# taylor-santos/RelativityPathTracer

Measured on AMD Instinct MI355X. Metric: Mrays/s (primary rays) on Scenes/bunny.txt at 3840x2160, higher is better.
Workload: dtype f32

## Files before the change

include/rpt.h:

```cpp
#ifndef RPT_H
#define RPT_H

#include "rpt_layout.h"

#ifdef __cplusplus
extern "C" {
#endif

typedef struct rpt_ctx rpt_ctx;

enum rpt_status {
    RPT_OK = 0,
    RPT_ERR_ARG = 1,
    RPT_ERR_STATE = 2,
    RPT_ERR_SCENE = 3,
    RPT_ERR_DEVICE = 4,
    RPT_ERR_NOMEM = 5
};

#define RPT_TILE_ROWS 8
#define RPT_LATENCY_KERNEL_MAX_PIXELS 3000000

const char *rpt_version(void);

// ... 39 lines not shown
int rpt_raymap_fill(int kind, const float *params, int width, int height, float *dirs3_out);

int rpt_set_environment(rpt_ctx *ctx, const unsigned char *rgb8, int width, int height);
int rpt_set_environment_frame(rpt_ctx *ctx, const float lorentz[16]);

int rpt_set_orientation(rpt_ctx *ctx, const float ypr[3]);
int rpt_set_field_of_view(rpt_ctx *ctx, float v_fov);
int rpt_orient_objects(const void *objects_in, int count, const float ypr[3], void *objects_out);
int rpt_orient_matrix(const float lorentz_in[16], const float ypr[3], float lorentz_out[16]);

int rpt_set_variant(rpt_ctx *ctx, int variant);
int rpt_set_msaa(rpt_ctx *ctx, int samples_per_axis);
int rpt_last_variant(const rpt_ctx *ctx);
int rpt_last_exact_rcp(const rpt_ctx *ctx);
int rpt_last_sky_split(const rpt_ctx *ctx, int rect[4]);
int rpt_scene_exact_rcp(const rpt_scene_desc *s);

int rpt_verify_frame(rpt_ctx *ctx, unsigned long long *differing_pixels);

int rpt_object_screen_rect(const void *object, int interval, const float *root_bounds_or_null, float rect_out[4]);
int rpt_object_screen_bounds(const void *object, int interval, const float *root_bounds_or_null, float bounds_out[8]);
int rpt_mesh_segment_cull_record(rpt_ctx *ctx, int object_index, float out[10]);
int rpt_object_screen_bounds_proposed(const void *object, int interval, const float *root_bounds_or_null, float bounds_out[8]);
int rpt_certify_screen_bounds(const void *object, int interval, const float *root_bounds_or_null, const float bounds[8], int stats_out[4]);
int rpt_tile_bitmap_host(const rpt_scene_desc *scene, int object_index, int interval, int width, int height, float lens_scale, int max_boxes,
                         const float *boxes_or_null, int n_boxes, uint32_t *bits_out, size_t words, int stats_out[5]);
int rpt_tile_bitmap_stage_host(const rpt_scene_desc *scene, int object_index, int interval, int width, int height, float lens_scale, int stage,
                               int max_triangles, uint32_t *bits_out, size_t words, int stats_out[4]);
int rpt_tile_rasterise_host(int width, int height, float lens_scale, int diagonals, const float bounds[8], uint32_t *bits_out, size_t words);
int rpt_tile_bitmap_state(rpt_ctx *ctx, unsigned long long out[4], int object_index, uint32_t *bits_or_null, size_t words);
// ... 152 lines not shown
```

relativitypathtracer_amd/_ffi.py:

```python
from __future__ import annotations

import ctypes as C
import os

_HERE = os.path.dirname(os.path.abspath(__file__))


class Float2(C.Structure):
    _fields_ = [("x", C.c_float), ("y", C.c_float)]


class Float4(C.Structure):
    _fields_ = [("x", C.c_float), ("y", C.c_float), ("z", C.c_float), ("w", C.c_float)]


class Object(C.Structure):
    _fields_ = [
        ("M", Float4 * 4), ("InvM", Float4 * 4), ("Lorentz", Float4 * 4), ("InvLorentz", Float4 * 4),
        ("stationaryCam", Float4), ("color", Float4),
        ("type", C.c_int32), ("meshIndex", C.c_int32), ("textureIndex", C.c_int32),
        ("textureWidth", C.c_int32), ("textureHeight", C.c_int32),
        ("light", C.c_uint8), ("_pad", C.c_uint8 * 3),
        ("flashPeriod", C.c_float), ("flashDuration", C.c_float),
    ]
# ... 133 lines not shown
    "rpt_object_screen_bounds_proposed": (C.c_int, [C.c_void_p, C.c_int, C.POINTER(C.c_float), C.POINTER(C.c_float)]),
    "rpt_certify_screen_bounds": (C.c_int, [C.c_void_p, C.c_int, C.POINTER(C.c_float), C.POINTER(C.c_float), C.POINTER(C.c_int)]),
    "rpt_tile_bitmap_host": (C.c_int, [C.c_void_p, C.c_int, C.c_int, C.c_int, C.c_int, C.c_float, C.c_int, C.c_void_p, C.c_int, C.c_void_p, C.c_size_t,
                                       C.POINTER(C.c_int)]),
    "rpt_tile_bitmap_stage_host": (C.c_int, [C.c_void_p, C.c_int, C.c_int, C.c_int, C.c_int, C.c_float, C.c_int, C.c_int, C.c_void_p, C.c_size_t,
                                             C.POINTER(C.c_int)]),
    "rpt_tile_rasterise_host": (C.c_int, [C.c_int, C.c_int, C.c_float, C.c_int, C.POINTER(C.c_float), C.c_void_p, C.c_size_t]),
    "rpt_tile_bitmap_shared_state": (C.c_int, [C.c_void_p, C.POINTER(C.c_uint64)]),
    "rpt_tile_bitmap_state": (C.c_int, [C.c_void_p, C.POINTER(C.c_uint64), C.c_int, C.c_void_p, C.c_size_t]),
    "rpt_derived_layout_host": (C.c_int, [C.c_void_p, C.c_int, C.c_void_p, C.c_size_t, C.POINTER(C.c_size_t)]),
    "rpt_probe_tile_masks": (C.c_int, [C.c_void_p, C.c_void_p, C.c_size_t]),
    "rpt_verify_frame": (C.c_int, [C.c_void_p, C.POINTER(C.c_uint64)]),
    "rpt_last_variant": (C.c_int, [C.c_void_p]),
    "rpt_last_exact_rcp": (C.c_int, [C.c_void_p]),
    "rpt_last_sky_split": (C.c_int, [C.c_void_p, C.POINTER(C.c_int)]),
    "rpt_scene_exact_rcp": (C.c_int, [C.c_void_p]),
    "rpt_probe_reciprocal": (C.c_int, [C.c_void_p, C.c_float, C.c_float, C.POINTER(C.c_uint64), C.c_void_p, C.c_int]),
    "rpt_set_msaa": (C.c_int, [C.c_void_p, C.c_int]),
    "rpt_probe_walk": (C.c_int, [C.c_void_p, C.c_int, C.c_void_p, C.c_void_p, C.c_int]),
    "rpt_timing_end_spans": (C.c_int, [C.c_void_p, C.c_void_p, C.POINTER(C.c_float), C.POINTER(C.c_float), C.c_int, C.POINTER(C.c_int)]),
    "rpt_probe_object": (C.c_int, [C.c_void_p, C.c_int, C.c_int, C.c_void_p, C.c_void_p, C.c_int]),
    "rpt_render": (C.c_int, [C.c_void_p]),
    "rpt_render_async": (C.c_int, [C.c_void_p]),
    "rpt_sync": (C.c_int, [C.c_void_p]),
    "rpt_output_ptr": (C.c_void_p, [C.c_void_p]),
    "rpt_output_bytes": (C.c_size_t, [C.c_void_p]),
    "rpt_read_framebuffer": (C.c_int, [C.c_void_p, C.c_void_p, C.c_size_t]),
    "rpt_read_debug_rgb": (C.c_int, [C.c_void_p, C.c_void_p, C.c_size_t]),
    "rpt_last_frame_ms": (C.c_int, [C.c_void_p, C.POINTER(C.c_float)]),
    "rpt_timed_frames": (C.c_int, [C.c_void_p, C.c_int, C.POINTER(C.c_float)]),
# ... 145 lines not shown
```

relativitypathtracer_amd/csrc/rpt_api.hip:

```cpp
#include <hip/hip_runtime.h>

#include <cmath>
#include <cstdio>
#include <chrono>
#include <cstdlib>
#include <cstring>
#include <algorithm>
#include <atomic>
#include <functional>
#include <map>
#include <memory>
#include <mutex>
#include <string>
#include <utility>
#include <vector>

#include "../../include/rpt.h"
#include "rpt_kernels.hip.h"
#include "rpt_octree_build.hip.h"
#include "rpt_screen_bounds.hpp"
#include "rpt_bounds_certify.hpp"
#include "rpt_tile_bitmap.hpp"
#include "rpt_sky_split.hpp"
#include "rpt_workers.hpp"
// ... 131 lines not shown
    DeviceBuffer tile_masks;
    DeviceBuffer verify_planes;
    DeviceBuffer claim_counters;
    int cu_count = 0;
    unsigned int claim_epoch = 0;
    std::vector<uint8_t> host_objects;
    DeviceBuffer dobjs;
    std::vector<rptb::Rect> rects;
    int rect_interval = 0x7fffffff;
    unsigned long long rect_geo_generation = ~0ull;
    DeviceBuffer owned_out, owned_plane, owned_rgb;
    void *pinned_objects = nullptr;
    size_t pinned_capacity = 0;
    hipEvent_t staging_done[4] = {nullptr, nullptr, nullptr, nullptr};
    unsigned int staging_used = 0, staging_next = 0;
    int object_count = 0;
    bool scene_uploaded = false;

    float white_point[3] = {1, 1, 1};
    float ambient = 1.0f;
    int width = 0, height = 0, interval = -1;
    bool params_set = false;

    void *external_out = nullptr;
    void *external_plane = nullptr;
    void *external_rgb = nullptr;
    std::vector<hipEvent_t> timing_events;
    int timing_frames = -1;
    bool want_owned_rgb = false;
    int first_tile = 0, tile_step = 1, run_log2 = 0;
// ... 756 lines not shown
    const long long want = (band + sky + 3) / 4;
    static const int wgs_per_cu = std::getenv("RPT_WGS_PER_CU") ? std::atoi(std::getenv("RPT_WGS_PER_CU")) : 5;
    const unsigned int wgs = (unsigned int)std::max(1ll, std::min((long long)ctx->cu_count * wgs_per_cu, want));
    switch (v) {
    case 60: hipLaunchKernelGGL(rptd::rpt_render_kernel_persistent_w5, dim3(wgs), dim3(256), 0, ctx->stream, a, a.out16, a.plane, a.debug_rgb, claims); break;
    case 62: hipLaunchKernelGGL(rptd::rpt_render_kernel_persistent_direct_w5, dim3(wgs), dim3(256), 0, ctx->stream, a, a.out16, a.plane, a.debug_rgb, claims); break;
    case 63: hipLaunchKernelGGL(rptd::rpt_render_kernel_persistent_classic_w5, dim3(wgs), dim3(256), 0, ctx->stream, a, a.out16, a.plane, a.debug_rgb, claims); break;
    default: return fail(ctx, RPT_ERR_ARG, "unknown persistent kernel variant");
    }
    return RPT_OK;
}
#endif

#ifdef RPT_DIAGNOSTICS
#define RPT_LAUNCH_X(N) case N: hipLaunchKernelGGL(rptd::rpt_render_kernel_x##N, grid, dim3(256), 0, ctx->stream, a); break;
void launch_sky_fill(rpt_ctx *ctx, const rptd::KernelArgs &a, int tiles, const int box[4]);
int launch_diagnostic(rpt_ctx *ctx, rptd::KernelArgs &a, dim3 grid, int tiles, int v) {
    if (v == 143 || v == 2573 || (v >= 256 && v < 1000 && (v & 8))) set_band_first(ctx, a, tiles);
    switch (v) {
    case 26: {
        const int tiles_x = ((ctx->width + 31) / 32) * 4;
        const int n_tiles = tiles_x * tiles;
        if (int rc = reserve(ctx, ctx->tile_masks, (size_t)n_tiles * 8)) return rc;
        a.mask_tiles_x = tiles_x;
        a.n_tiles = n_tiles;
        a.tile_masks = (unsigned long long *)ctx->tile_masks.ptr;
        hipLaunchKernelGGL(rptd::rpt_tile_bin_kernel, dim3((n_tiles + 255) / 256), dim3(256), 0, ctx->stream, a);
        hipLaunchKernelGGL(rptd::rpt_render_kernel_v1_masked_w5, grid, dim3(256), 0, ctx->stream, a);
        break;
    }
    case 40: hipLaunchKernelGGL(rptd::rpt_render_kernel_ballot_w4, dim3(grid.x * 4, grid.y), dim3(64), 0, ctx->stream, a); break;
// ... 13 lines not shown
    case 2257: hipLaunchKernelGGL(rptd::rpt_render_kernel_x257_w4, grid, dim3(256), 0, ctx->stream, a); break;
    case 2259: hipLaunchKernelGGL(rptd::rpt_render_kernel_x259_w4, grid, dim3(256), 0, ctx->stream, a); break;
    case 2263: hipLaunchKernelGGL(rptd::rpt_render_kernel_x263_w4, grid, dim3(256), 0, ctx->stream, a); break;
    RPT_LAUNCH_X(689) RPT_LAUNCH_X(701)
    case 2573: hipLaunchKernelGGL(rptd::rpt_render_kernel_x573_w4, grid, dim3(256), 0, ctx->stream, a); break;
    case 7:
        if (int rc = reserve(ctx, ctx->counters, 16 * sizeof(unsigned long long))) return rc;
        RPT_HIP(ctx, hipMemsetAsync(ctx->counters.ptr, 0, 16 * sizeof(unsigned long long), ctx->stream));
        a.counters = (unsigned long long *)ctx->counters.ptr;
        hipLaunchKernelGGL(rptd::rpt_render_kernel_v1_diag, grid, dim3(256), 0, ctx->stream, a);
        break;
    case 8: hipLaunchKernelGGL(rptd::rpt_render_kernel_primary_only, grid, dim3(256), 0, ctx->stream, a); break;
    case 786: {
        if (!a.out16) return fail(ctx, RPT_ERR_ARG, "variant 786 writes the 16-byte framebuffer only");
        const int no_box[4] = {0, 0, 0, 0};
        launch_sky_fill(ctx, a, tiles, no_box);
        break;
    }
    case 11:
        if (int rc = reserve(ctx, ctx->wave_times, (size_t)grid.x * grid.y * 4 * 10 * sizeof(unsigned long long))) return rc;
        RPT_HIP(ctx, hipMemsetAsync(ctx->wave_times.ptr, 0, ctx->wave_times.bytes, ctx->stream));
        a.wave_times = (unsigned long long *)ctx->wave_times.ptr;
        hipLaunchKernelGGL(rptd::rpt_render_kernel_v1_timeline, grid, dim3(256), 0, ctx->stream, a);
        break;
    default: return fail(ctx, RPT_ERR_ARG, "unknown kernel variant");
    }
    return RPT_OK;
}
#endif

bool projection_params(const float *params, float out[3]) {
// ... 491 lines not shown
    if (int rc = staged_host(ctx, ctx->tile_bits, bytes, &host)) return rc;
    bool any = false;
    for (int i = 0; i < slots; i++) {
        if (!(todo >> i & 1ull)) continue;
        const auto t0 = std::chrono::steady_clock::now();
        if (!shared_tile_bitmap(ctx, objs[i], (uint32_t *)host + (size_t)i * words)) continue;
        ctx->bits_last_build_us = std::chrono::duration<double, std::micro>(std::chrono::steady_clock::now() - t0).count();
        ctx->bits_has |= 1ull << i;
        ctx->bits_builds++;
        any = true;
    }
    if (any) return staged_copy(ctx, ctx->tile_bits);
    return RPT_OK;
}

void fill_frame_args(const rpt_ctx *ctx, rptd::LensArgs &a) {
    std::memset((void *)&a, 0, sizeof a);
    a.dnodes = (const rptd::DNode *)ctx->geo->dnodes.ptr;
    a.dtris = (const rptd::DTri *)ctx->geo->dtris.ptr;
    a.links = (const int *)ctx->geo->dlinks.ptr;
    a.first_tris = (const rptd::DTri *)ctx->geo->dfirst.ptr;
    a.exits = (const rptd::DExit *)ctx->geo->dexits.ptr;
    a.hits = (const rptd::DHit *)ctx->geo->dhits.ptr;
    a.top_count = ctx->geo->top_count;
    a.dobjs = (const rptd::DObj *)((const char *)ctx->objects.ptr + (size_t)ctx->object_count * sizeof(rpt_object));
    a.objects = (const rpt_object *)ctx->objects.ptr;
    a.rects = (const float4 *)((const char *)ctx->objects.ptr + (size_t)ctx->object_count * (sizeof(rpt_object) + sizeof(rptd::DObj)));
    a.vertices = (const rpt_float3 *)ctx->geo->vertices.ptr;
    a.normals = (const rpt_float3 *)ctx->geo->normals.ptr;
    a.uvs = (const rpt_float2 *)ctx->geo->uvs.ptr;
// ... 58 lines not shown
              !rptd::tile_origin_policy<rptd::DopplerTwin<rptd::BallotExact>> && !rptd::tile_origin_policy<rptd::Lens<rptd::BallotExact>>,
              "the forms sky_split_box lets through (walk, analytic, ieee) are the kernels that add tile_x0");
bool sky_split_box(const rpt_ctx *ctx, const Choice &c, Call call, const rptd::KernelArgs &a, int tiles, int box[4]) {
    const KernelRow *row = c.colour;
    if (!row || !row->kernel || c.windowed || c.refine || row->camera != Camera::pinhole || row->colour != Colour::plain) return false;
    if (!(row->form == Form::walk || row->form == Form::analytic || row->form == Form::ieee)) return false;
    if (call.kind != CallKind::in_flight || (long long)ctx->width * ctx->height <= ctx->sky_split_min_pixels) return false;
    if (!a.out16 || a.plane || a.debug_rgb || ctx->colour_plane || ctx->first_tile != 0 || ctx->tile_step != 1 || ctx->run_log2 != 0) return false;
    if (ctx->msaa > 1 || ctx->doppler || ctx->env_on || ctx->v_fov != 0.0f || ctx->projection != RPT_PROJECTION_PINHOLE) return false;
    if (ctx->object_count < 1 || ctx->object_count > 64 || ctx->rects.size() != (size_t)ctx->object_count) return false;
    if (!rpts::object_box(ctx->rects.data(), ctx->object_count, ctx->width, ctx->height, box)) return false;
    const long long tiles_x = (ctx->width + 7) / 8, covered = (long long)(box[2] - box[0]) * (box[3] - box[1]);
    return covered * 100 <= tiles_x * tiles * ctx->sky_split_share;
}

void launch_sky_fill(rpt_ctx *ctx, const rptd::KernelArgs &a, int tiles, const int box[4]) {
    rptd::SkyFillArgs s;
    s.out16 = a.out16;
    s.width = ctx->width;
    s.height = ctx->height;
    s.bg_packed = a.bg_packed;
    s.tx0 = box[0]; s.ty0 = box[1]; s.tx1 = box[2]; s.ty1 = box[3];
    const int tiles_x = (ctx->width + 7) / 8;
    hipLaunchKernelGGL(rptd::rpt_sky_fill_kernel, dim3((tiles_x + RPT_SKY_FILL_TILES - 1) / RPT_SKY_FILL_TILES, tiles), dim3(64), 0, ctx->stream, s);
}

int launch(rpt_ctx *ctx, Call call) {
    const Choice c = choose_kernels(ctx, call);
    if (call.colour_frame && ctx->scene_uploaded && ctx->params_set) ctx->last_aa_variant = 0;
    if (c.code != RPT_OK) return fail(ctx, c.code, c.text);
    ctx->last_sky_split = false;
    if (int rc = ensure_outputs(ctx)) return rc;
    const int tiles = local_tile_count(ctx);
    if (call.colour_frame && ctx->aa_n > 1) {
        if (int rc = reserve(ctx, ctx->aa_plane, (size_t)tiles * RPT_TILE_ROWS * ctx->width * 4)) return rc;
        if (int rc = tally_ready(ctx, ctx->tally[TALLY_AA], 1)) return rc;
    }
    if (c.nothing) return RPT_OK;
    const bool panorama = ctx->projection == RPT_PROJECTION_EQUIRECT;
// ... 13 lines not shown
    a.msaa = ctx->msaa;
    a.doppler = ctx->doppler;
    a.debug_doppler = doppler_recording(ctx) ? (float *)(ctx->external_doppler ? ctx->external_doppler : ctx->owned_doppler.ptr) : nullptr;
    ctx->doppler_recorded = a.debug_doppler != nullptr;
    a.env_texels = ctx->env_on ? (const uint32_t *)ctx->env.device.ptr : nullptr;
    a.env_width = ctx->env_width;
    a.env_height = ctx->env_height;
    std::memcpy(a.env_frame, ctx->env_frame, sizeof a.env_frame);
    if (ctx->oriented) {
        rpt_float4 e[4];
        std::memcpy(e, ctx->env_frame, sizeof e);
        rebase_columns(e, ctx->R, a.env_frame);
    }

    const dim3 grid1(((ctx->width + 31) / 32) * 4, tiles);
    if (!c.colour) {
#ifdef RPT_DIAGNOSTICS
        const dim3 grid((ctx->width + 31) / 32, tiles);
        if (int rc = launch_diagnostic(ctx, a, grid, tiles, c.variant)) return rc;
#endif
    } else if (!c.colour->kernel) {
        if (rpt_launch_relaxed_kernel(relaxed_waves(c.colour->form), &a, sizeof(rptd::KernelArgs), grid1.x, grid1.y, (void *)ctx->stream)) return fail(ctx, RPT_ERR_DEVICE, "relaxed-arithmetic kernel launch failed");
    } else {
        dim3 grid = grid1;
        int box[4];
        if (sky_split_box(ctx, c, call, a, tiles, box)) {
            launch_sky_fill(ctx, a, tiles, box);
            a.tile_x0 = box[0];
            a.first_tile = box[1];
            grid = dim3(box[2] - box[0], box[3] - box[1]);
            ctx->last_sky_split = true;
            std::memcpy(ctx->last_sky_box, box, sizeof box);
        }
        void *args[] = {(void *)&a};
        (void)hipLaunchKernel(c.kernel(c.launched()), grid, dim3(64), args, 0, ctx->stream);
    }
    RPT_HIP(ctx, hipGetLastError());
    ctx->last_variant = c.variant;
    ctx->last_exact_rcp = c.ran_exact(c.launched());
    Tally &refined = ctx->tally[TALLY_AA];
    if (c.refine) {
        rptd::RefineArgs ra;
// ... 16 lines not shown
        tally_off(refined);
    }
    return RPT_OK;
}

int launch_events(rpt_ctx *ctx) {
    const Choice c = choose_kernels(ctx, Call{CallKind::events, false});
    if (c.code != RPT_OK) return fail(ctx, c.code, c.text);
    const size_t px = (size_t)ctx->width * ctx->height;
    if (!ctx->external_events && (px * sizeof(rpt_event) > ctx->owned_events.capacity || ctx->owned_events.bytes != px * sizeof(rpt_event))) {
        if (int rc = reserve(ctx, ctx->owned_events, px * sizeof(rpt_event))) return rc;
        RPT_HIP(ctx, hipMemsetAsync(ctx->owned_events.ptr, 0, px * sizeof(rpt_event), ctx->stream));
    }
    if (ctx->projection == RPT_PROJECTION_EQUIRECT)
        if (int rc = ensure_projection_tables(ctx, ctx->pano, 1)) return rc;
    rptd::RaymapEventArgs ea;
    std::memset((void *)&ea, 0, sizeof ea);
    fill_frame_args(ctx, ea);
    ea.raymap = c.colour->camera == Camera::raymap ? (const float4 *)ctx->raymap.device.ptr : nullptr;
    ea.raymap_pitch = ctx->raymap_pitch;
    ea.out16 = nullptr;
    ea.plane = nullptr;
    ea.debug_rgb = nullptr;
    ea.events = (rpt_event *)(ctx->external_events ? ctx->external_events : ctx->owned_events.ptr);
    ctx->event_frame.buffer = ea.events;
    ctx->event_frame.width = ctx->width;
    ctx->event_frame.height = ctx->height;
    ctx->events_first_tile = ctx->first_tile;
    ctx->events_tile_step = ctx->tile_step;
    ctx->events_run_log2 = ctx->run_log2;
// ... 31 lines not shown
    *out16_out = out16;
    *events_out = events;
    return RPT_OK;
}

using PassEnqueue = int (*)(rpt_ctx *ctx, Tally &tally, rpt_pixel *out16, const rpt_event *events);
int frame_pass(rpt_ctx *ctx, const char *call, bool on, int which, PassEnqueue enqueue) {
    Tally &tally = ctx->tally[which];
    if (!on) {
        tally_off(tally);
        return RPT_OK;
    }
    rpt_pixel *out16 = nullptr;
    const rpt_event *events = nullptr;
    if (int rc = frames_of_this_view(ctx, call, &out16, &events)) return rc;
    if (int rc = enqueue(ctx, tally, out16, events)) return rc;
    if (int rc = tally_home(ctx, tally)) return rc;
    ctx->last_event = tally.copied;
    return RPT_OK;
}

int enqueue_overlay(rpt_ctx *ctx, Tally &tally, rpt_pixel *out16, const rpt_event *events) {
    const rpt_overlay_desc &d = ctx->overlay;
    if (int rc = tally_ready(ctx, tally, 1, 8)) return rc;

    rptd::OverlayArgs a;
    std::memset(&a, 0, sizeof a);
    a.events = events;
    a.out16 = out16;
    a.changed = (unsigned long long *)tally.device.ptr;
// ... 405 lines not shown
const char *rpt_version(void) { return "rpt-hip 0.2 (gfx950)"; }
#endif

int rpt_create(rpt_ctx **out, int device_ordinal) {
    if (!out) return RPT_ERR_ARG;
    *out = nullptr;
    int n = 0;
    if (hipGetDeviceCount(&n) != hipSuccess || n <= 0) return RPT_ERR_DEVICE;
    if (device_ordinal < 0 || device_ordinal >= n) return RPT_ERR_ARG;
    rpt_ctx *ctx = new (std::nothrow) rpt_ctx();
    if (!ctx) return RPT_ERR_NOMEM;
    ctx->device = device_ordinal;
    ctx->tile_triangles = tile_triangles_wanted();
    ctx->sky_split_share = sky_split_share_wanted();
    ctx->sky_split_min_pixels = sky_split_min_pixels_wanted();
    (void)rpth::Workers::instance();
    {
        static std::atomic<int> created{0};
        ctx->serial = created.fetch_add(1);
    }
    ctx->geo = std::make_shared<Geometry>();
    ctx->geo->device = device_ordinal;
    if (hipSetDevice(device_ordinal) != hipSuccess || hipStreamCreateWithFlags(&ctx->own_stream, hipStreamNonBlocking) != hipSuccess ||

        hipEventCreate(&ctx->ev_begin) != hipSuccess || hipEventCreate(&ctx->ev_end) != hipSuccess) {
        rpt_destroy(ctx);
        return RPT_ERR_DEVICE;
    }
    ctx->stream = ctx->own_stream;
    if (hipDeviceGetAttribute(&ctx->cu_count, hipDeviceAttributeMultiprocessorCount, device_ordinal) != hipSuccess || ctx->cu_count <= 0) ctx->cu_count = 256;
// ... 114 lines not shown
    std::vector<uint8_t> &given = ctx->given_scratch, &turned = ctx->turned_scratch;
    given.assign((const uint8_t *)objects, (const uint8_t *)objects + bytes);
    turned.resize(bytes);
    orient_objects((const rpt_object *)given.data(), count, ctx->R, (rpt_object *)turned.data());
    const int rc = set_objects_as_given(ctx, turned.data(), count);
    if (rc == RPT_OK) ctx->caller_objects.swap(given);
    return rc;
}

static int set_objects_as_given(rpt_ctx *ctx, const void *objects, int count) {
    if (!ctx->scene_uploaded) return fail(ctx, RPT_ERR_STATE, "rpt_set_objects before rpt_upload_scene");
    RPT_HIP(ctx, hipSetDevice(ctx->device));
    if (int rc = validate_objects(ctx, (const rpt_object *)objects, count)) return rc;
    const size_t bytes = (size_t)count * sizeof(rpt_object);
    const size_t dbytes = (size_t)count * (sizeof(rptd::DObj) + sizeof(rptb::Rect));
    const size_t slot_bytes = ((bytes + dbytes + 255) / 256) * 256;
    if (slot_bytes * RPT_STAGING_SLOTS > ctx->pinned_capacity) {
        RPT_HIP(ctx, hipStreamSynchronize(ctx->stream));
        if (ctx->pinned_objects) RPT_HIP(ctx, hipHostFree(ctx->pinned_objects));
        ctx->pinned_objects = nullptr;
        ctx->pinned_capacity = 0;
        const size_t cap = (slot_bytes < 4096 ? 4096 : slot_bytes * 2) * RPT_STAGING_SLOTS;
        RPT_HIP(ctx, hipHostMalloc(&ctx->pinned_objects, cap, hipHostMallocDefault));
        ctx->pinned_capacity = cap;
        for (int k = 0; k < RPT_STAGING_SLOTS; k++)
            if (!ctx->staging_done[k]) RPT_HIP(ctx, hipEventCreateWithFlags(&ctx->staging_done[k], hipEventDisableTiming));
        ctx->staging_used = 0;
    }
    if (bytes + dbytes > ctx->objects.capacity) RPT_HIP(ctx, hipStreamSynchronize(ctx->stream));
    if (int rc = reserve(ctx, ctx->objects, bytes + dbytes)) return rc;
    if (bytes) {
        const int k = (int)(ctx->staging_next % RPT_STAGING_SLOTS);
        RPT_HOST_MARK(0);
        if (ctx->staging_used & (1u << k)) RPT_HIP(ctx, hipEventSynchronize(ctx->staging_done[k]));
        RPT_HOST_MARK(1);
        char *slot = (char *)ctx->pinned_objects + (ctx->pinned_capacity / RPT_STAGING_SLOTS) * k;
        std::memcpy(slot, objects, bytes);
        build_dobjs(ctx, (const rpt_object *)objects, count, (rptd::DObj *)(slot + bytes));
        if (ctx->windows.size() == 2 * (size_t)count)
            for (int i = 0; i < count; i++) {
                rptd::DObj &d = ((rptd::DObj *)(slot + bytes))[i];
                d.win_t0 = ctx->windows[2 * (size_t)i];
                d.win_t1 = ctx->windows[2 * (size_t)i + 1];
            }
        RPT_HOST_MARK(2);
        note_still_objects(ctx, (const rpt_object *)objects, count);
        build_rects(ctx, (const rpt_object *)objects, count, (rptb::Rect *)(slot + bytes + (size_t)count * sizeof(rptd::DObj)));
        RPT_HOST_MARK(3);
        RPT_HIP(ctx, hipMemcpyAsync(ctx->objects.ptr, slot, bytes + dbytes, hipMemcpyHostToDevice, ctx->stream));
        RPT_HOST_MARK(4);
        RPT_HIP(ctx, hipEventRecord(ctx->staging_done[k], ctx->stream));
        RPT_HOST_MARK(5);
        ctx->last_event = ctx->staging_done[k];
        ctx->staging_used |= 1u << k;
        ctx->staging_next++;
    }
    if (!bytes) ctx->bits_still = ctx->bits_tried = ctx->bits_has = 0;
    ctx->object_count = count;
    ctx->has_mesh = false;
    for (int i = 0; i < count; i++) ctx->has_mesh = ctx->has_mesh || ((const rpt_object *)objects)[i].type == RPT_MESH;
    ctx->host_objects.assign((const uint8_t *)objects, (const uint8_t *)objects + bytes);
    ctx->view_generation++;
    return RPT_OK;
}

int rpt_set_params(rpt_ctx *ctx, const float white_point[3], float ambient, int width, int height, int interval) {
    if (!ctx || !white_point) return RPT_ERR_ARG;
    if (width <= 0 || height <= 0 || (long long)width * height > (1ll << 31) - 1) return fail(ctx, RPT_ERR_ARG, "rpt_set_params: bad resolution");
    for (int c = 0; c < 3; c++) ctx->white_point[c] = white_point[c];
    ctx->ambient = ambient;
    ctx->width = width;
    ctx->height = height;
// ... 451 lines not shown
    if (!ctx || !out) return RPT_ERR_ARG;
    std::lock_guard<std::mutex> lock(ctx->geo->bitmap_cache_lock);
    out[0] = ctx->geo->bitmap_builds;
    out[1] = ctx->geo->bitmap_copies;
    return RPT_OK;
}

int rpt_probe_tile_masks(rpt_ctx *ctx, unsigned long long *out, size_t tiles) {
    if (!ctx || !out) return RPT_ERR_ARG;
    if (!ctx->scene_uploaded || !ctx->params_set) return fail(ctx, RPT_ERR_STATE, "rpt_probe_tile_masks before rpt_upload_scene / rpt_set_params");
    if (ctx->projection != RPT_PROJECTION_PINHOLE || !window_holds_frame(ctx)) return fail(ctx, RPT_ERR_ARG, "rpt_probe_tile_masks: this frame is not rendered with the object mask");
    const int tx = (ctx->width + 7) / 8, ty = (ctx->height + 7) / 8;
    if (tiles != (size_t)tx * ty) return fail(ctx, RPT_ERR_ARG, "rpt_probe_tile_masks: tiles != ceil(width / 8) * ceil(height / 8)");
    RPT_HIP(ctx, hipSetDevice(ctx->device));
    if (int rc = ensure_tile_bits(ctx)) return rc;
    rptd::LensArgs a;
    fill_frame_args(ctx, a);
    unsigned long long *d_out = nullptr;
    RPT_HIP(ctx, hipMalloc((void **)&d_out, tiles * 16));
    hipLaunchKernelGGL(rptd::rpt_probe_tile_masks_kernel, dim3(tx, ty), dim3(64), 0, ctx->stream, a, ctx->v_fov != 0.0f ? 1 : 0, d_out);
    hipError_t e = hipGetLastError();
    if (e == hipSuccess) e = hipMemcpyAsync(out, d_out, tiles * 16, hipMemcpyDeviceToHost, ctx->stream);
    if (e == hipSuccess) e = hipStreamSynchronize(ctx->stream);
    (void)hipFree(d_out);
    if (e != hipSuccess) return fail(ctx, RPT_ERR_DEVICE, std::string("rpt_probe_tile_masks: ") + hipGetErrorString(e));
    return RPT_OK;
}

int rpt_set_variant(rpt_ctx *ctx, int variant) {
    if (!ctx) return RPT_ERR_ARG;
#ifndef RPT_DIAGNOSTICS
    if (variant != 0 && settable_form(variant) == Form::diagnostic)
        return fail(ctx, RPT_ERR_ARG, "rpt_set_variant: unknown variant (measurement arms and instrumented kernels exist in librpt_hip_diag.so only)");
#endif
    ctx->variant = variant;
    return RPT_OK;
}

int rpt_last_variant(const rpt_ctx *ctx) { return ctx ? ctx->last_variant : 0; }
int rpt_last_exact_rcp(const rpt_ctx *ctx) { return ctx && ctx->last_exact_rcp ? 1 : 0; }
int rpt_last_sky_split(const rpt_ctx *ctx, int rect[4]) {
    const bool split = ctx && ctx->last_sky_split;
    if (rect)
        for (int k = 0; k < 4; k++) rect[k] = split ? ctx->last_sky_box[k] : 0;
    return split ? 1 : 0;
}

int rpt_scene_exact_rcp(const rpt_scene_desc *s) {
    if (!s || (s->vertex_count && !s->vertices) || (s->triangle_words && !s->triangles) || (s->octree_tri_count && !s->octreeTris)) return -RPT_ERR_ARG;
    const size_t n_tris = s->triangle_words / RPT_TRI_STRIDE;
    const double limit = 0x1p60;
    for (size_t i = 0; i < s->octree_tri_count; i++) {
        const int t = s->octreeTris[i];
        if (t < 0 || (size_t)t >= n_tris) return -RPT_ERR_SCENE;
        const rpt_float3 *vv[3];
        for (int c = 0; c < 3; c++) {
            const uint32_t w = s->triangles[9 * (size_t)t + 3 * c];
            if (w >= s->vertex_count) return -RPT_ERR_SCENE;
            vv[c] = &s->vertices[w];
        }
// ... 602 lines not shown
            rc = fail(ctx, RPT_ERR_DEVICE, "rpt_probe: device error");
    }
    (void)hipFree(d_in);
    (void)hipFree(d_out);
    return rc;
}

int rpt_probe_walk(rpt_ctx *ctx, int object_index, const float *host_rays, float *host_out, int n) {
    if (!ctx || !host_rays || !host_out || n <= 0) return RPT_ERR_ARG;
    if (!ctx->scene_uploaded || ctx->object_count <= 0) return fail(ctx, RPT_ERR_STATE, "rpt_probe_walk before rpt_upload_scene / rpt_set_objects");
    if (object_index < 0 || object_index >= ctx->object_count || ctx->host_objects.size() < (size_t)(object_index + 1) * sizeof(rpt_object) ||
        ((const rpt_object *)ctx->host_objects.data())[object_index].type != RPT_MESH)
        return fail(ctx, RPT_ERR_ARG, "rpt_probe_walk: not a mesh object");
    if (!ctx->geo->compact_ok) return fail(ctx, RPT_ERR_STATE, "rpt_probe_walk: this octree has no derived layout (children not consecutive)");
    RPT_HIP(ctx, hipSetDevice(ctx->device));
    rptd::KernelArgs a;
    probe_kernel_args(ctx, a);
    float *d_in = nullptr, *d_out = nullptr;
    RPT_HIP(ctx, hipMalloc((void **)&d_in, sizeof(float) * 6 * (size_t)n));
    if (hipMalloc((void **)&d_out, sizeof(float) * 24 * (size_t)n) != hipSuccess) {
        (void)hipFree(d_in);
        return fail(ctx, RPT_ERR_NOMEM, "rpt_probe_walk: hipMalloc");
    }
    int rc = RPT_OK;
    if (hipMemcpy(d_in, host_rays, sizeof(float) * 6 * (size_t)n, hipMemcpyHostToDevice) != hipSuccess) rc = RPT_ERR_DEVICE;
    if (!rc) {
        hipLaunchKernelGGL(rptd::rpt_probe_walk_kernel, dim3((n + 255) / 256), dim3(256), 0, ctx->stream, a, object_index, d_in, d_out, n,
                           ctx->geo->exact_rcp_ok ? 1 : 0);
        if (hipGetLastError() != hipSuccess || hipStreamSynchronize(ctx->stream) != hipSuccess ||
            hipMemcpy(host_out, d_out, sizeof(float) * 24 * (size_t)n, hipMemcpyDeviceToHost) != hipSuccess)
// ... 28 lines not shown
            hipMemcpy(counts_out, d_counts, 5 * sizeof(unsigned long long), hipMemcpyDeviceToHost) != hipSuccess ||
            (d_samples && hipMemcpy(samples_out, d_samples, sizeof(float) * 2 * (size_t)max_samples, hipMemcpyDeviceToHost) != hipSuccess))
            rc = fail(ctx, RPT_ERR_DEVICE, "rpt_probe_reciprocal: device error");
    }
    (void)hipFree(d_counts);
    if (d_samples) (void)hipFree(d_samples);
    return rc;
}

int rpt_probe_object(rpt_ctx *ctx, int which, int object_index, const float *host_in, float *host_out, int n) {
    if (!ctx || !host_in || !host_out || n <= 0 || which < 0 || which > 3) return RPT_ERR_ARG;
    if (!ctx->scene_uploaded || ctx->object_count <= 0) return fail(ctx, RPT_ERR_STATE, "rpt_probe_object before rpt_upload_scene / rpt_set_objects");
    if (object_index < 0 || object_index >= ctx->object_count) return fail(ctx, RPT_ERR_ARG, "rpt_probe_object: no such object");
    if (!ctx->geo->compact_ok) return fail(ctx, RPT_ERR_STATE, "rpt_probe_object: this octree has no derived layout (children not consecutive)");
    RPT_HIP(ctx, hipSetDevice(ctx->device));
    rptd::KernelArgs a;
    probe_kernel_args(ctx, a);
    const size_t in_floats = which == 0 ? 8 : which == 1 ? 9 : which == 2 ? 4 : 3, out_floats = which == 1 ? 2 : which == 2 ? 16 : 8;
    float *d_in = nullptr, *d_out = nullptr;
    RPT_HIP(ctx, hipMalloc((void **)&d_in, sizeof(float) * in_floats * (size_t)n));
    if (hipMalloc((void **)&d_out, sizeof(float) * out_floats * (size_t)n) != hipSuccess) {
        (void)hipFree(d_in);
        return fail(ctx, RPT_ERR_NOMEM, "rpt_probe_object: hipMalloc");
    }
    int rc = RPT_OK;
    if (hipMemcpy(d_in, host_in, sizeof(float) * in_floats * (size_t)n, hipMemcpyHostToDevice) != hipSuccess) rc = RPT_ERR_DEVICE;
    if (!rc) {
        hipLaunchKernelGGL(rptd::rpt_probe_object_kernel, dim3((n + 63) / 64), dim3(64), 0, ctx->stream, a, which, object_index, d_in, d_out, n);
        if (hipGetLastError() != hipSuccess || hipStreamSynchronize(ctx->stream) != hipSuccess ||
            hipMemcpy(host_out, d_out, sizeof(float) * out_floats * (size_t)n, hipMemcpyDeviceToHost) != hipSuccess)
// ... 235 lines not shown
```

relativitypathtracer_amd/csrc/rpt_kernels.hip.h:

```cpp
#pragma once
#include "../../include/rpt_layout.h"
#include "rpt_device_math.hip.h"

#ifdef RPT_RELAXED_FP
#pragma clang fp contract(fast)
#else
#pragma clang fp contract(off)
#endif

namespace rptd {

#define RPT_EPSILON 0.0000001f
#define RPT_MAX_LEAF_STEPS 4096
#define RPT_LINK_CHILD_MASK 0x00ffffff
#define RPT_TOP_MAX 3072
#define RPT_PI_D 3.14159265358979323846264338327950288

struct alignas(64) DNode {
    float minx, miny, minz; int link;
    float maxx, maxy, maxz; int leafBegin;
    int leafCount; int nb[6]; int pad;
};
static_assert(sizeof(DNode) == 64, "DNode is one 64-B line");
struct alignas(16) DTri { float ax, ay, az, e1x; float e1y, e1z, e2x, e2y; float e2z; int tri; int pad0, pad1; };
// ... 1343 lines not shown
__global__ __launch_bounds__(64) void rpt_render_kernel_v0(const KernelArgs a) { render_pixel_body<RefLayout>(a); }
__global__ __launch_bounds__(64) __attribute__((amdgpu_waves_per_eu(5, 5))) void rpt_render_kernel_unculled_w5(const KernelArgs a) { render_pixel_body<Unculled>(a); }
__global__ __launch_bounds__(64) __attribute__((amdgpu_waves_per_eu(5, 5))) void rpt_render_kernel_ballot_w5(const KernelArgs a) { render_pixel_body<BallotExact>(a); }
__global__ __launch_bounds__(64) __attribute__((amdgpu_waves_per_eu(5, 5))) void rpt_render_kernel_ballot_first_w5(const KernelArgs a) { render_pixel_body<BallotFirstExact>(a); }
__global__ __launch_bounds__(64) __attribute__((amdgpu_waves_per_eu(5, 5))) void rpt_render_kernel_ballot_ieee_w5(const KernelArgs a) { render_pixel_body<Ballot>(a); }
__global__ __launch_bounds__(64) __attribute__((amdgpu_waves_per_eu(5, 5))) void rpt_render_kernel_ballot_first_ieee_w5(const KernelArgs a) { render_pixel_body<BallotFirst>(a); }
__global__ __launch_bounds__(64) __attribute__((amdgpu_waves_per_eu(8, 8))) void rpt_render_kernel_analytic_w8(const KernelArgs a) { render_pixel_body<Analytic>(a); }

#define RPT_SKY_FILL_TILES 8
struct SkyFillArgs {
    rpt_pixel *out16;
    int width, height;
    uint32_t bg_packed;
    int tx0, ty0, tx1, ty1;
};
__global__ __launch_bounds__(64) __attribute__((amdgpu_waves_per_eu(8, 8))) void rpt_sky_fill_kernel(const SkyFillArgs a) {
    const int lane = threadIdx.x & 63;
    const int ty = (int)blockIdx.y, tx_first = (int)blockIdx.x * RPT_SKY_FILL_TILES;
    const bool box_rows = ty >= a.ty0 && ty < a.ty1;
    if (box_rows && tx_first >= a.tx0 && tx_first + RPT_SKY_FILL_TILES <= a.tx1) return;
    const int y = ty * RPT_TILE_ROWS + (lane >> 3);
    if (y >= a.height) return;
    const uint32_t fy = __float_as_uint((float)y);
    const size_t row = (size_t)y * a.width;
#pragma unroll
    for (int k = 0; k < RPT_SKY_FILL_TILES; k++) {
        const int tx = tx_first + k, x = tx * 8 + (lane & 7);
        const bool in_box = box_rows && tx >= a.tx0 && tx < a.tx1;
        if (!in_box && x < a.width) store_pixel(a.out16, row + x, __float_as_uint((float)x), fy, a.bg_packed, 0u);
    }
}

__global__ __launch_bounds__(64) __attribute__((amdgpu_waves_per_eu(5, 5))) void rpt_render_kernel_msaa_w5(const KernelArgs a) { render_pixel_body_msaa<Ballot>(a); }
__global__ __launch_bounds__(64) __attribute__((amdgpu_waves_per_eu(5, 5))) void rpt_render_kernel_msaa_unculled_w5(const KernelArgs a) { render_pixel_body_msaa<Unculled>(a); }

__global__ __launch_bounds__(64) __attribute__((amdgpu_waves_per_eu(5, 5))) void rpt_render_kernel_unculled_doppler_w5(const DopplerArgs a) { render_pixel_body<DopplerTwin<Unculled>>(a); }
__global__ __launch_bounds__(64) __attribute__((amdgpu_waves_per_eu(5, 5))) void rpt_render_kernel_ballot_doppler_w5(const DopplerArgs a) { render_pixel_body<DopplerTwin<BallotExact>>(a); }
__global__ __launch_bounds__(64) __attribute__((amdgpu_waves_per_eu(5, 5))) void rpt_render_kernel_ballot_first_doppler_w5(const DopplerArgs a) { render_pixel_body<DopplerTwin<BallotFirstExact>>(a); }
__global__ __launch_bounds__(64) __attribute__((amdgpu_waves_per_eu(5, 5))) void rpt_render_kernel_ballot_ieee_doppler_w5(const DopplerArgs a) { render_pixel_body<DopplerTwin<Ballot>>(a); }
__global__ __launch_bounds__(64) __attribute__((amdgpu_waves_per_eu(5, 5))) void rpt_render_kernel_ballot_first_ieee_doppler_w5(const DopplerArgs a) { render_pixel_body<DopplerTwin<BallotFirst>>(a); }
__global__ __launch_bounds__(64) __attribute__((amdgpu_waves_per_eu(8, 8))) void rpt_render_kernel_analytic_doppler_w8(const DopplerArgs a) { render_pixel_body<DopplerTwin<Analytic>>(a); }
__global__ __launch_bounds__(64) __attribute__((amdgpu_waves_per_eu(5, 5))) void rpt_render_kernel_doppler_record_w5(const DopplerArgs a) { render_pixel_body<DopplerRecorded>(a); }

__global__ __launch_bounds__(64) __attribute__((amdgpu_waves_per_eu(5, 5))) void rpt_render_kernel_pano_w5(const PanoramaArgs a) { render_pixel_body<PanoramaWalk>(a); }
__global__ __launch_bounds__(64) __attribute__((amdgpu_waves_per_eu(5, 5))) void rpt_render_kernel_pano_ieee_w5(const PanoramaArgs a) { render_pixel_body<PanoramaWalkIeee>(a); }
// ... 768 lines not shown
```

relativitypathtracer_amd/renderer.py:

```python
from __future__ import annotations

import ctypes as C
import math
from typing import Mapping, Optional, Sequence, Tuple, Union

import numpy as np

from . import _ffi
from .events import EVENT_DTYPE
from .scene import Scene

PIXEL_DTYPE = np.dtype([("x", "<f4"), ("y", "<f4"), ("rgba", "u1", (4,)), ("unspecified", "<u4")])
TILE_ROWS = 8
DOPPLER_SHIFT, DOPPLER_BEAMING = 1, 2
DOPPLER_RECORD = 11
PROJECTIONS = {"pinhole": 0, "equirect": 1, "raymap": 2}
RAYMAP_KINDS = {"fisheye": 0, "equisolid": 1, "stereographic": 2, "cube_strip": 3}


class RenderError(RuntimeError):
    code = None


def _projection_args(mode: str, h_fov: float, v_fov: float, yaw: float):
# ... 265 lines not shown

    def read_debug_doppler(self) -> np.ndarray:
        out = np.empty((self.height, self.width, DOPPLER_RECORD), dtype=np.float32)
        self._check(self._lib.rpt_read_debug_doppler(self._h, out.ctypes.data, out.nbytes), "rpt_read_debug_doppler")
        return out

    def last_variant(self) -> int:
        return int(self._lib.rpt_last_variant(self._h))

    def last_exact_rcp(self) -> bool:
        return bool(self._lib.rpt_last_exact_rcp(self._h))

    def last_sky_split(self) -> Optional[Tuple[int, int, int, int]]:
        box = (C.c_int * 4)()
        return tuple(int(v) for v in box) if self._lib.rpt_last_sky_split(self._h, box) else None

    def verify_frame(self) -> int:
        n = C.c_uint64(0)
        self._check(self._lib.rpt_verify_frame(self._h, C.byref(n)), "rpt_verify_frame")
        return int(n.value)

    def render(self):
        self._check(self._lib.rpt_render(self._h), "rpt_render")

    def render_async(self):
        self._check(self._lib.rpt_render_async(self._h), "rpt_render_async")

    def sync(self):
        self._check(self._lib.rpt_sync(self._h), "rpt_sync")

# ... 422 lines not shown
```

Baseline: 123,000.

## Pass small object tables as kernel arguments instead of pinned staging copies

When the per-frame object data (objects, device objects, rects) fits in 3840 bytes, it is staged into a host block and delivered as a kernel argument. A copy kernel writes it, or the sky-fill kernel's first block writes it when a sky split runs. This removes the hipMemcpyAsync, the event record and the possible host wait on a staging slot each frame. In exchange it adds a tiny kernel launch or a larger argument payload, and it changes ordering assumptions for object buffer consumers.

After: 121,700. -1.1%, worse.

```diff
diff --git a/include/rpt.h b/include/rpt.h
--- a/include/rpt.h
+++ b/include/rpt.h
@@ -77,6 +77,12 @@
 int rpt_last_variant(const rpt_ctx *ctx);
 int rpt_last_exact_rcp(const rpt_ctx *ctx);
 int rpt_last_sky_split(const rpt_ctx *ctx, int rect[4]);
+#define RPT_OBJECTS_PATH_NONE 0
+#define RPT_OBJECTS_PATH_STAGING 1
+#define RPT_OBJECTS_PATH_KERNEL 2
+#define RPT_OBJECTS_PATH_FILL 3
+int rpt_last_objects_path(const rpt_ctx *ctx);
+int rpt_read_object_block(rpt_ctx *ctx, void *host_dst, size_t bytes, size_t *bytes_needed);
 int rpt_scene_exact_rcp(const rpt_scene_desc *s);
 
 int rpt_verify_frame(rpt_ctx *ctx, unsigned long long *differing_pixels);
diff --git a/relativitypathtracer_amd/_ffi.py b/relativitypathtracer_amd/_ffi.py
--- a/relativitypathtracer_amd/_ffi.py
+++ b/relativitypathtracer_amd/_ffi.py
@@ -171,6 +171,8 @@
     "rpt_last_variant": (C.c_int, [C.c_void_p]),
     "rpt_last_exact_rcp": (C.c_int, [C.c_void_p]),
     "rpt_last_sky_split": (C.c_int, [C.c_void_p, C.POINTER(C.c_int)]),
+    "rpt_last_objects_path": (C.c_int, [C.c_void_p]),
+    "rpt_read_object_block": (C.c_int, [C.c_void_p, C.c_void_p, C.c_size_t, C.POINTER(C.c_size_t)]),
     "rpt_scene_exact_rcp": (C.c_int, [C.c_void_p]),
     "rpt_probe_reciprocal": (C.c_int, [C.c_void_p, C.c_float, C.c_float, C.POINTER(C.c_uint64), C.c_void_p, C.c_int]),
     "rpt_set_msaa": (C.c_int, [C.c_void_p, C.c_int]),
diff --git a/relativitypathtracer_amd/csrc/rpt_api.hip b/relativitypathtracer_amd/csrc/rpt_api.hip
--- a/relativitypathtracer_amd/csrc/rpt_api.hip
+++ b/relativitypathtracer_amd/csrc/rpt_api.hip
@@ -169,6 +169,11 @@
     size_t pinned_capacity = 0;
     hipEvent_t staging_done[4] = {nullptr, nullptr, nullptr, nullptr};
     unsigned int staging_used = 0, staging_next = 0;
+    rptk::PendingObjectBlock object_block;
+    bool object_block_on = true;
+    bool objects_staged = false;
+    int last_objects_path = 0;
+    size_t device_block_bytes = 0;
     int object_count = 0;
     bool scene_uploaded = false;
 
@@ -955,7 +960,7 @@
 
 #ifdef RPT_DIAGNOSTICS
 #define RPT_LAUNCH_X(N) case N: hipLaunchKernelGGL(rptd::rpt_render_kernel_x##N, grid, dim3(256), 0, ctx->stream, a); break;
-void launch_sky_fill(rpt_ctx *ctx, const rptd::KernelArgs &a, int tiles, const int box[4]);
+int launch_sky_fill(rpt_ctx *ctx, const rptd::KernelArgs &a, int tiles, const int box[4]);
 int launch_diagnostic(rpt_ctx *ctx, rptd::KernelArgs &a, dim3 grid, int tiles, int v) {
     if (v == 143 || v == 2573 || (v >= 256 && v < 1000 && (v & 8))) set_band_first(ctx, a, tiles);
     switch (v) {
@@ -999,7 +1004,7 @@
     case 786: {
         if (!a.out16) return fail(ctx, RPT_ERR_ARG, "variant 786 writes the 16-byte framebuffer only");
         const int no_box[4] = {0, 0, 0, 0};
-        launch_sky_fill(ctx, a, tiles, no_box);
+        if (int rc = launch_sky_fill(ctx, a, tiles, no_box)) return rc;
         break;
     }
     case 11:
@@ -1521,6 +1526,36 @@
     return RPT_OK;
 }
 
+static_assert(sizeof(rptd::ObjectBlock) == sizeof(rptk::PendingObjectBlock::bytes) && (sizeof(rpt_object) + sizeof(rptd::DObj) + sizeof(rptb::Rect)) % 16 == 0,
+              "the pending block is the kernels' argument, in whole 16-byte words per object");
+static_assert(sizeof(rptd::SkyFillBlockArgs) <= 4096, "a kernel's arguments: 4 KB");
+bool object_block_args(rpt_ctx *ctx, rptd::ObjectBlockArgs &b) {
+    const rptk::PendingObjectBlock &p = ctx->object_block;
+    if (!p.pending() || p.words > RPT_OBJECT_BLOCK_WORDS || (size_t)p.words * 16 > ctx->objects.capacity || !ctx->objects.ptr) return false;
+    b.dst = (uint4 *)ctx->objects.ptr;
+    b.words = (int)p.words;
+    std::memcpy(&b.block, p.bytes, sizeof b.block);
+    return true;
+}
+void object_block_delivered(rpt_ctx *ctx, int path) {
+    if (ctx->object_block.pending()) ctx->device_block_bytes = (size_t)ctx->object_block.words * 16;
+    ctx->object_block.clear();
+    ctx->objects_staged = false;
+    ctx->last_objects_path = path;
+}
+int deliver_object_block(rpt_ctx *ctx) {
+    if (!ctx->object_block.pending()) {
+        object_block_delivered(ctx, ctx->objects_staged ? RPT_OBJECTS_PATH_STAGING : RPT_OBJECTS_PATH_NONE);
+        return RPT_OK;
+    }
+    rptd::ObjectBlockArgs b;
+    if (!object_block_args(ctx, b)) return fail(ctx, RPT_ERR_STATE, "the pending object block does not fit the context's object buffer");
+    hipLaunchKernelGGL(rptd::rpt_object_block_kernel, dim3(1), dim3(64), 0, ctx->stream, b);
+    RPT_HIP(ctx, hipGetLastError());
+    object_block_delivered(ctx, RPT_OBJECTS_PATH_KERNEL);
+    return RPT_OK;
+}
+
 void fill_frame_args(const rpt_ctx *ctx, rptd::LensArgs &a) {
     std::memset((void *)&a, 0, sizeof a);
     a.dnodes = (const rptd::DNode *)ctx->geo->dnodes.ptr;
@@ -1609,15 +1644,24 @@
     return covered * 100 <= tiles_x * tiles * ctx->sky_split_share;
 }
 
-void launch_sky_fill(rpt_ctx *ctx, const rptd::KernelArgs &a, int tiles, const int box[4]) {
-    rptd::SkyFillArgs s;
+int launch_sky_fill(rpt_ctx *ctx, const rptd::KernelArgs &a, int tiles, const int box[4]) {
+    rptd::SkyFillBlockArgs sb;
+    rptd::SkyFillArgs &s = sb.fill;
     s.out16 = a.out16;
     s.width = ctx->width;
     s.height = ctx->height;
     s.bg_packed = a.bg_packed;
     s.tx0 = box[0]; s.ty0 = box[1]; s.tx1 = box[2]; s.ty1 = box[3];
     const int tiles_x = (ctx->width + 7) / 8;
-    hipLaunchKernelGGL(rptd::rpt_sky_fill_kernel, dim3((tiles_x + RPT_SKY_FILL_TILES - 1) / RPT_SKY_FILL_TILES, tiles), dim3(64), 0, ctx->stream, s);
+    const dim3 grid((tiles_x + RPT_SKY_FILL_TILES - 1) / RPT_SKY_FILL_TILES, tiles);
+    if (!ctx->object_block.pending()) {
+        hipLaunchKernelGGL(rptd::rpt_sky_fill_kernel, grid, dim3(64), 0, ctx->stream, s);
+        return RPT_OK;
+    }
+    if (!object_block_args(ctx, sb.objects)) return fail(ctx, RPT_ERR_STATE, "the pending object block does not fit the context's object buffer");
+    hipLaunchKernelGGL(rptd::rpt_sky_fill_block_kernel, grid, dim3(64), 0, ctx->stream, sb);
+    object_block_delivered(ctx, RPT_OBJECTS_PATH_FILL);
+    return RPT_OK;
 }
 
 int launch(rpt_ctx *ctx, Call call) {
@@ -1661,6 +1705,10 @@
     }
 
     const dim3 grid1(((ctx->width + 31) / 32) * 4, tiles);
+    int box[4];
+    const bool split = sky_split_box(ctx, c, call, a, tiles, box);
+    if (!split || !ctx->object_block.pending())
+        if (int rc = deliver_object_block(ctx)) return rc;
     if (!c.colour) {
 #ifdef RPT_DIAGNOSTICS
         const dim3 grid((ctx->width + 31) / 32, tiles);
@@ -1670,9 +1718,8 @@
         if (rpt_launch_relaxed_kernel(relaxed_waves(c.colour->form), &a, sizeof(rptd::KernelArgs), grid1.x, grid1.y, (void *)ctx->stream)) return fail(ctx, RPT_ERR_DEVICE, "relaxed-arithmetic kernel launch failed");
     } else {
         dim3 grid = grid1;
-        int box[4];
-        if (sky_split_box(ctx, c, call, a, tiles, box)) {
-            launch_sky_fill(ctx, a, tiles, box);
+        if (split) {
+            if (int rc = launch_sky_fill(ctx, a, tiles, box)) return rc;
             a.tile_x0 = box[0];
             a.first_tile = box[1];
             grid = dim3(box[2] - box[0], box[3] - box[1]);
@@ -1719,6 +1766,7 @@
     }
     if (ctx->projection == RPT_PROJECTION_EQUIRECT)
         if (int rc = ensure_projection_tables(ctx, ctx->pano, 1)) return rc;
+    if (int rc = deliver_object_block(ctx)) return rc;
     rptd::RaymapEventArgs ea;
     std::memset((void *)&ea, 0, sizeof ea);
     fill_frame_args(ctx, ea);
@@ -1780,6 +1828,7 @@
     rpt_pixel *out16 = nullptr;
     const rpt_event *events = nullptr;
     if (int rc = frames_of_this_view(ctx, call, &out16, &events)) return rc;
+    if (int rc = deliver_object_block(ctx)) return rc;
     if (int rc = enqueue(ctx, tally, out16, events)) return rc;
     if (int rc = tally_home(ctx, tally)) return rc;
     ctx->last_event = tally.copied;
@@ -2215,6 +2264,7 @@
     ctx->tile_triangles = tile_triangles_wanted();
     ctx->sky_split_share = sky_split_share_wanted();
     ctx->sky_split_min_pixels = sky_split_min_pixels_wanted();
+    ctx->object_block_on = env_integer("RPT_OBJECT_BLOCK", 0, 1, 1) != 0;
     (void)rpth::Workers::instance();
     {
         static std::atomic<int> created{0};
@@ -2359,8 +2409,10 @@
     if (int rc = validate_objects(ctx, (const rpt_object *)objects, count)) return rc;
     const size_t bytes = (size_t)count * sizeof(rpt_object);
     const size_t dbytes = (size_t)count * (sizeof(rptd::DObj) + sizeof(rptb::Rect));
+    const rptk::ObjectBlockLayout layout = rptk::object_block_layout((size_t)count, sizeof(rpt_object), sizeof(rptd::DObj), sizeof(rptb::Rect));
+    const bool rides = ctx->object_block_on && rptk::object_block_rides(layout);
     const size_t slot_bytes = ((bytes + dbytes + 255) / 256) * 256;
-    if (slot_bytes * RPT_STAGING_SLOTS > ctx->pinned_capacity) {
+    if (!rides && slot_bytes * RPT_STAGING_SLOTS > ctx->pinned_capacity) {
         RPT_HIP(ctx, hipStreamSynchronize(ctx->stream));
         if (ctx->pinned_objects) RPT_HIP(ctx, hipHostFree(ctx->pinned_objects));
         ctx->pinned_objects = nullptr;
@@ -2377,9 +2429,10 @@
     if (bytes) {
         const int k = (int)(ctx->staging_next % RPT_STAGING_SLOTS);
         RPT_HOST_MARK(0);
-        if (ctx->staging_used & (1u << k)) RPT_HIP(ctx, hipEventSynchronize(ctx->staging_done[k]));
+        if (!rides && (ctx->staging_used & (1u << k))) RPT_HIP(ctx, hipEventSynchronize(ctx->staging_done[k]));
         RPT_HOST_MARK(1);
-        char *slot = (char *)ctx->pinned_objects + (ctx->pinned_capacity / RPT_STAGING_SLOTS) * k;
+        char *slot = rides ? (char *)ctx->object_block.stage(layout)
+                           : (char *)ctx->pinned_objects + (ctx->pinned_capacity / RPT_STAGING_SLOTS) * k;
         std::memcpy(slot, objects, bytes);
         build_dobjs(ctx, (const rpt_object *)objects, count, (rptd::DObj *)(slot + bytes));
         if (ctx->windows.size() == 2 * (size_t)count)
@@ -2392,15 +2445,29 @@
         note_still_objects(ctx, (const rpt_object *)objects, count);
         build_rects(ctx, (const rpt_object *)objects, count, (rptb::Rect *)(slot + bytes + (size_t)count * sizeof(rptd::DObj)));
         RPT_HOST_MARK(3);
-        RPT_HIP(ctx, hipMemcpyAsync(ctx->objects.ptr, slot, bytes + dbytes, hipMemcpyHostToDevice, ctx->stream));
-        RPT_HOST_MARK(4);
-        RPT_HIP(ctx, hipEventRecord(ctx->staging_done[k], ctx->stream));
-        RPT_HOST_MARK(5);
-        ctx->last_event = ctx->staging_done[k];
-        ctx->staging_used |= 1u << k;
-        ctx->staging_next++;
-    }
-    if (!bytes) ctx->bits_still = ctx->bits_tried = ctx->bits_has = 0;
+        if (!rides) {
+            ctx->object_block.clear();
+            RPT_HIP(ctx, hipMemcpyAsync(ctx->objects.ptr, slot, bytes + dbytes, hipMemcpyHostToDevice, ctx->stream));
+            RPT_HOST_MARK(4);
+            RPT_HIP(ctx, hipEventRecord(ctx->staging_done[k], ctx->stream));
+            RPT_HOST_MARK(5);
+            ctx->last_event = ctx->staging_done[k];
+            ctx->staging_used |= 1u << k;
+            ctx->staging_next++;
+            ctx->objects_staged = true;
+            ctx->device_block_bytes = bytes + dbytes;
+            ctx->last_objects_path = RPT_OBJECTS_PATH_STAGING;
+        } else {
+            RPT_HOST_MARK(4);
+            RPT_HOST_MARK(5);
+        }
+    }
+    if (!bytes) {
+        ctx->bits_still = ctx->bits_tried = ctx->bits_has = 0;
+        ctx->object_block.clear();
+        ctx->device_block_bytes = 0;
+        ctx->objects_staged = false;
+    }
     ctx->object_count = count;
     ctx->has_mesh = false;
     for (int i = 0; i < count; i++) ctx->has_mesh = ctx->has_mesh || ((const rpt_object *)objects)[i].type == RPT_MESH;
@@ -2882,6 +2949,7 @@
     if (tiles != (size_t)tx * ty) return fail(ctx, RPT_ERR_ARG, "rpt_probe_tile_masks: tiles != ceil(width / 8) * ceil(height / 8)");
     RPT_HIP(ctx, hipSetDevice(ctx->device));
     if (int rc = ensure_tile_bits(ctx)) return rc;
+    if (int rc = deliver_object_block(ctx)) return rc;
     rptd::LensArgs a;
     fill_frame_args(ctx, a);
     unsigned long long *d_out = nullptr;
@@ -2912,6 +2980,19 @@
     if (rect)
         for (int k = 0; k < 4; k++) rect[k] = split ? ctx->last_sky_box[k] : 0;
     return split ? 1 : 0;
+}
+
+int rpt_last_objects_path(const rpt_ctx *ctx) { return ctx ? ctx->last_objects_path : 0; }
+
+int rpt_read_object_block(rpt_ctx *ctx, void *host_dst, size_t bytes, size_t *bytes_needed) {
+    if (!ctx || (bytes && !host_dst)) return RPT_ERR_ARG;
+    RPT_HIP(ctx, hipSetDevice(ctx->device));
+    RPT_HIP(ctx, hipStreamSynchronize(ctx->stream));
+    const size_t have = ctx->device_block_bytes <= ctx->objects.capacity ? ctx->device_block_bytes : 0;
+    if (bytes_needed) *bytes_needed = have;
+    const size_t n = bytes < have ? bytes : have;
+    if (n) RPT_HIP(ctx, hipMemcpy(host_dst, ctx->objects.ptr, n, hipMemcpyDeviceToHost));
+    return RPT_OK;
 }
 
 int rpt_scene_exact_rcp(const rpt_scene_desc *s) {
@@ -3544,6 +3625,7 @@
         return fail(ctx, RPT_ERR_ARG, "rpt_probe_walk: not a mesh object");
     if (!ctx->geo->compact_ok) return fail(ctx, RPT_ERR_STATE, "rpt_probe_walk: this octree has no derived layout (children not consecutive)");
     RPT_HIP(ctx, hipSetDevice(ctx->device));
+    if (int rc = deliver_object_block(ctx)) return rc;
     rptd::KernelArgs a;
     probe_kernel_args(ctx, a);
     float *d_in = nullptr, *d_out = nullptr;
@@ -3602,6 +3684,7 @@
     if (object_index < 0 || object_index >= ctx->object_count) return fail(ctx, RPT_ERR_ARG, "rpt_probe_object: no such object");
     if (!ctx->geo->compact_ok) return fail(ctx, RPT_ERR_STATE, "rpt_probe_object: this octree has no derived layout (children not consecutive)");
     RPT_HIP(ctx, hipSetDevice(ctx->device));
+    if (int rc = deliver_object_block(ctx)) return rc;
     rptd::KernelArgs a;
     probe_kernel_args(ctx, a);
     const size_t in_floats = which == 0 ? 8 : which == 1 ? 9 : which == 2 ? 4 : 3, out_floats = which == 1 ? 2 : which == 2 ? 16 : 8;
diff --git a/relativitypathtracer_amd/csrc/rpt_kernels.hip.h b/relativitypathtracer_amd/csrc/rpt_kernels.hip.h
--- a/relativitypathtracer_amd/csrc/rpt_kernels.hip.h
+++ b/relativitypathtracer_amd/csrc/rpt_kernels.hip.h
@@ -1,6 +1,7 @@
 #pragma once
 #include "../../include/rpt_layout.h"
 #include "rpt_device_math.hip.h"
+#include "rpt_object_block.hpp"
 
 #ifdef RPT_RELAXED_FP
 #pragma clang fp contract(fast)
@@ -1381,7 +1382,7 @@
     uint32_t bg_packed;
     int tx0, ty0, tx1, ty1;
 };
-__global__ __launch_bounds__(64) __attribute__((amdgpu_waves_per_eu(8, 8))) void rpt_sky_fill_kernel(const SkyFillArgs a) {
+__device__ __forceinline__ void sky_fill_body(const SkyFillArgs a) {
     const int lane = threadIdx.x & 63;
     const int ty = (int)blockIdx.y, tx_first = (int)blockIdx.x * RPT_SKY_FILL_TILES;
     const bool box_rows = ty >= a.ty0 && ty < a.ty1;
@@ -1396,6 +1397,28 @@
         const bool in_box = box_rows && tx >= a.tx0 && tx < a.tx1;
         if (!in_box && x < a.width) store_pixel(a.out16, row + x, __float_as_uint((float)x), fy, a.bg_packed, 0u);
     }
+}
+__global__ __launch_bounds__(64) __attribute__((amdgpu_waves_per_eu(8, 8))) void rpt_sky_fill_kernel(const SkyFillArgs a) { sky_fill_body(a); }
+
+struct ObjectBlock {
+    uint4 w[RPT_OBJECT_BLOCK_WORDS];
+};
+__device__ __forceinline__ void store_object_block(const ObjectBlock &block, uint4 *dst, int words) {
+    for (int i = (int)(threadIdx.x & 63); i < words && i < RPT_OBJECT_BLOCK_WORDS; i += 64) dst[i] = block.w[i];
+}
+struct ObjectBlockArgs {
+    uint4 *dst;
+    int words;
+    ObjectBlock block;
+};
+__global__ __launch_bounds__(64) void rpt_object_block_kernel(const ObjectBlockArgs a) { store_object_block(a.block, a.dst, a.words); }
+struct SkyFillBlockArgs {
+    SkyFillArgs fill;
+    ObjectBlockArgs objects;
+};
+__global__ __launch_bounds__(64) __attribute__((amdgpu_waves_per_eu(8, 8))) void rpt_sky_fill_block_kernel(const SkyFillBlockArgs a) {
+    if (blockIdx.x == 0 && blockIdx.y == 0) store_object_block(a.objects.block, a.objects.dst, a.objects.words);
+    sky_fill_body(a.fill);
 }
 
 __global__ __launch_bounds__(64) __attribute__((amdgpu_waves_per_eu(5, 5))) void rpt_render_kernel_msaa_w5(const KernelArgs a) { render_pixel_body_msaa<Ballot>(a); }
diff --git a/relativitypathtracer_amd/csrc/rpt_object_block.hpp b/relativitypathtracer_amd/csrc/rpt_object_block.hpp
--- /dev/null
+++ b/relativitypathtracer_amd/csrc/rpt_object_block.hpp
@@ -0,0 +1,40 @@
+#pragma once
+#include <cstddef>
+#include <cstdint>
+#include <cstring>
+
+#define RPT_OBJECT_BLOCK_BYTES 3840
+#define RPT_OBJECT_BLOCK_WORDS (RPT_OBJECT_BLOCK_BYTES / 16)
+
+namespace rptk {
+
+struct ObjectBlockLayout {
+    size_t dobjs = 0, rects = 0, bytes = 0;
+};
+
+inline ObjectBlockLayout object_block_layout(size_t count, size_t object_bytes, size_t dobj_bytes, size_t rect_bytes) {
+    ObjectBlockLayout l;
+    l.dobjs = count * object_bytes;
+    l.rects = l.dobjs + count * dobj_bytes;
+    l.bytes = l.rects + count * rect_bytes;
+    return l;
+}
+
+inline bool object_block_rides(const ObjectBlockLayout &l) { return l.bytes > 0 && l.bytes % 16 == 0 && l.bytes <= RPT_OBJECT_BLOCK_BYTES; }
+
+struct PendingObjectBlock {
+    alignas(16) unsigned char bytes[RPT_OBJECT_BLOCK_BYTES];
+    unsigned int words = 0;
+
+    PendingObjectBlock() { std::memset(bytes, 0, sizeof bytes); }
+    bool pending() const { return words != 0; }
+    void clear() { words = 0; }
+    unsigned char *stage(const ObjectBlockLayout &l) {
+        if (!object_block_rides(l)) return nullptr;
+        std::memset(bytes + l.bytes, 0, sizeof bytes - l.bytes);
+        words = (unsigned int)(l.bytes / 16);
+        return bytes;
+    }
+};
+
+}
diff --git a/relativitypathtracer_amd/renderer.py b/relativitypathtracer_amd/renderer.py
--- a/relativitypathtracer_amd/renderer.py
+++ b/relativitypathtracer_amd/renderer.py
@@ -303,6 +303,17 @@
     def last_sky_split(self) -> Optional[Tuple[int, int, int, int]]:
         box = (C.c_int * 4)()
         return tuple(int(v) for v in box) if self._lib.rpt_last_sky_split(self._h, box) else None
+
+    def last_objects_path(self) -> int:
+        return int(self._lib.rpt_last_objects_path(self._h))
+
+    def read_object_block(self) -> np.ndarray:
+        need = C.c_size_t(0)
+        self._check(self._lib.rpt_read_object_block(self._h, None, 0, C.byref(need)), "rpt_read_object_block")
+        out = np.zeros(int(need.value), dtype=np.uint8)
+        if out.size:
+            self._check(self._lib.rpt_read_object_block(self._h, out.ctypes.data, out.size, None), "rpt_read_object_block")
+        return out
 
     def verify_frame(self) -> int:
         n = C.c_uint64(0)
```
